# SkylerGao/MC_NeRF

Hardware: AMD Instinct MI355X
Metric: train rays/sec (coarse+fine, 64+128 samples) (higher is better)
Workload: dtype f16x3h; 1 GPU; Ball_Lego-shaped 110-view 800x800, coarse 4x128 @64 + fine 8x256 @128-grid, GLOBAL_OPTIM stage, fwd+bwd+allreduce+RAdam; precision=f16x3h, parallelism=dp1

## Files before the change

### mc_nerf_amd/csrc/mcnerf_16.h

```cpp
#pragma once
#include "mcnerf_common.h"

#define MCN16_SLAB 16
#define MCN16_RING (128 / MCN16_SLAB)
#define MCN16_AHEAD (MCN16_RING - 2)
#define MCN16_PPW (MCN16_SLAB / 8)
#define MCN16_WAVES 8
#define MCN16_ROWS (32 * MCN16_WAVES)
#define MCN16_ENCKS 4

struct Mcn16Part { int src, ld, col0, out_real, con_real, ksteps, map; };
static inline __host__ __device__ int mcn16_map_enc(int map) { return map >= 1 && map <= MCN_NFREQ; }
struct Mcn16Seg { int first_frag, tiles, transposed; Mcn16Part a, b; };
#define MCN16_MAXSEG 24
struct Mcn16Stream { int nseg, total_frags; Mcn16Seg seg[MCN16_MAXSEG]; };

static inline int mcn16_pad(int frags) { return (frags + MCN16_SLAB - 1) / MCN16_SLAB * MCN16_SLAB; }

static inline void mcn16_add(Mcn16Stream& st, int tiles, int transposed, Mcn16Part a, Mcn16Part b) {
    Mcn16Seg& s = st.seg[st.nseg++];
    s.first_frag = st.total_frags; s.tiles = tiles; s.transposed = transposed; s.a = a; s.b = b;
    st.total_frags += mcn16_pad(tiles * (a.ksteps + b.ksteps));
}

static inline Mcn16Stream mcn16_fwd_stream(const McnLayout& L) {
    Mcn16Stream st; st.nseg = 0; st.total_frags = 0;
    const int W = L.width, NT = W / 32, KS = W / 16;
    const int ME = L.nfreq == MCN_NFREQ ? 0 : L.nfreq, MS = L.sh_deg == 2 ? 0 : 16 + L.sh_deg;
    const Mcn16Part none = {0, 0, 0, 0, 0, 0, 0};
    mcn16_add(st, NT, 0, Mcn16Part{L.pW[0], L.nenc, 0, W, MCN_ENC, MCN16_ENCKS, ME}, none);
    for (int l = 1; l < L.depth; ++l) {
        if (l == L.skip) mcn16_add(st, NT, 0, Mcn16Part{L.pW[l], W + L.nenc, 0, W, MCN_ENC, MCN16_ENCKS, ME},
                                   Mcn16Part{L.pW[l], W + L.nenc, L.nenc, W, W, KS, 0});
        else mcn16_add(st, NT, 0, Mcn16Part{L.pW[l], W, 0, W, W, KS, 0}, none);
    }
    mcn16_add(st, NT, 0, Mcn16Part{L.pWs1, W, 0, W, W, KS, 0}, none);
    mcn16_add(st, NT, 0, Mcn16Part{L.pWc1, W, 0, W, W, KS, 0}, none);
    mcn16_add(st, 1, 0, Mcn16Part{L.pWc2, W, 0, MCN_NSH, W, KS, MS}, none);
    return st;
}
static inline Mcn16Stream mcn16_bwd_stream(const McnLayout& L) {
    Mcn16Stream st; st.nseg = 0; st.total_frags = 0;
    const int W = L.width, NT = W / 32, KS = W / 16;
    const int ME = L.nfreq == MCN_NFREQ ? 0 : L.nfreq, MS = L.sh_deg == 2 ? 0 : 16 + L.sh_deg;
    const Mcn16Part none = {0, 0, 0, 0, 0, 0, 0};
    mcn16_add(st, NT, 1, Mcn16Part{L.pWs1, W, 0, W, W, KS, 0}, none);
    mcn16_add(st, NT, 1, Mcn16Part{L.pWc2, W, 0, W, MCN_NSH, 2, MS}, none);
    mcn16_add(st, NT, 1, Mcn16Part{L.pWc1, W, 0, W, W, KS, 0}, none);
    for (int l = L.depth - 1; l >= 1; --l) {
        const int ld = (l == L.skip) ? W + L.nenc : W;
        if (l == L.skip) mcn16_add(st, 2, 1, Mcn16Part{L.pW[l], ld, 0, MCN_ENC, W, KS, ME}, none);
        mcn16_add(st, NT, 1, Mcn16Part{L.pW[l], ld, (l == L.skip) ? L.nenc : 0, W, W, KS, 0}, none);
    }
    mcn16_add(st, 2, 1, Mcn16Part{L.pW[0], L.nenc, 0, MCN_ENC, W, KS, ME}, none);
    return st;
}

static inline long long mcn16_cap_tiles(long long capacity) { return (capacity + MCN16_ROWS - 1) / MCN16_ROWS * MCN16_WAVES; }
static inline size_t mcn16_slot_bytes(long long capacity, int width) { return (size_t)mcn16_cap_tiles(capacity) * (width / 16) * 1024; }
static inline int mcn16_mask_words(int width) { return width >= 64 ? width / 64 : 1; }
static inline size_t mcn16_mask_slot_bytes(long long capacity, int width) { return (size_t)mcn16_cap_tiles(capacity) * 64 * 4 * mcn16_mask_words(width); }
static inline size_t mcn16_enc_bytes(long long capacity) { return (size_t)mcn16_cap_tiles(capacity) * MCN16_ENCKS * 1024; }
static inline size_t mcn16_dsh_bytes(long long capacity) { return (size_t)mcn16_cap_tiles(capacity) * 2 * 1024; }

static inline bool mcn16_is_bf16(int dtype) { return dtype == 1; }
static inline bool mcn16_x3_chain(int dtype) { return dtype == 2 || dtype == 3; }
static inline bool mcn16_hi_planes_only(int dtype) { return dtype == 3; }

struct Mcn16FwdArgs {
    McnLayout lay;
    const float* params;
    const void* packed;
    int stream_slabs;
    int dtype;
    const float* rays_o; const float* rays_d; const float* zgrid; const float* jitter; const float* barf_w;
    const int2* idx; const int* count; int max_rows; int n_rays, S;
    float* out;
    void* act_ws; size_t slot_bytes;
    void* enc_ws;
    unsigned* mask_ws; size_t mask_slot_words;
    void* sh_ws;
    int z_stride = 0;
};
hipError_t mcn16_launch_fwd(const Mcn16FwdArgs& a, hipStream_t st);

struct Mcn16BwdArgs {
    McnLayout lay;
    const float* params;
    const void* packed;
    int stream_slabs;
    int dtype;
    const float* rays_o; const float* rays_d; const float* zgrid; const float* jitter; const float* barf_w;
    const int2* idx; const int* count; int max_rows; int n_rays, S;
    const float* out; const float* d_out;
    const unsigned* mask_ws; size_t mask_slot_words;
    const void* enc_ws;
    const void* sh_ws;
    void* dy_ws; size_t slot_bytes;
    void* dsh_ws;
    float* d_rays_o; float* d_rays_d;
    const unsigned* gmax_bits;
    int z_stride = 0;
};
hipError_t mcn16_launch_bwd(const Mcn16BwdArgs& a, hipStream_t st);

struct Mcn16DwArgs {
    McnLayout lay;
    int dtype;
    const int* count; int rows;
    const void* act_ws; const void* enc_ws; const void* dy_ws; const void* dsh_ws;
    size_t slot_bytes;
    float* grads;
    const unsigned* gmax_bits;
    float x_scale;
};
hipError_t mcn16_launch_dw(const Mcn16DwArgs& a, hipStream_t st);

struct Dw16Seg {
    const char* dY; int ksn;
    const char* X;  int ksk;
    const char* X2; int ksk2;
    int n_lo, n_real;
    int col, k_real;
    int col2, k_real2;
    float* dW; int ldw;
    float* db;
    int kmap, kmap2, nmap;
};
#define MCN16_DW_MAXSEG 15

template <class Job>
static inline bool mcn16_dw_job(const Mcn16DwArgs& a, Job& job) {
    const McnLayout& L = a.lay;
    const int W = L.width, D = L.depth, KS = W / 16;
    const int ME = L.nfreq == MCN_NFREQ ? 0 : L.nfreq, MS = L.sh_deg == 2 ? 0 : 16 + L.sh_deg;
    auto act = [&](int slot) { return reinterpret_cast<const char*>(a.act_ws) + (size_t)slot * a.slot_bytes; };
    auto dy = [&](int slot) { return reinterpret_cast<const char*>(a.dy_ws) + (size_t)slot * a.slot_bytes; };
    const char* dsh = reinterpret_cast<const char*>(a.dsh_ws);
    float* const g = a.grads;
    job.n = 0;
    if (D + 5 > MCN16_DW_MAXSEG) return false;
    auto add = [&](int shape, const char* dY, int ksn, int n_lo, int n_real, float* dW, int ldw, float* db, int nmap = 0) -> Dw16Seg& {
        Dw16Seg& s = job.seg[job.n];
        job.shape[job.n++] = shape;
        s = Dw16Seg{};
        s.dY = dY; s.ksn = ksn; s.n_lo = n_lo; s.n_real = n_real; s.dW = dW; s.ldw = ldw; s.db = db; s.nmap = nmap;
        return s;
    };
    auto input = [](Dw16Seg& s, const char* x, int ks, int col, int k_real, int kmap) {
        if (!s.X) { s.X = x; s.ksk = ks; s.col = col; s.k_real = k_real; s.kmap = kmap; }
        else { s.X2 = x; s.ksk2 = ks; s.col2 = col; s.k_real2 = k_real; s.kmap2 = kmap; }
    };
    auto hidden = [&](Dw16Seg& s, int slot, int col) { input(s, act(slot), KS, col, W, 0); };
    auto encoded = [&](Dw16Seg& s) { input(s, reinterpret_cast<const char*>(a.enc_ws), MCN16_ENCKS, 0, MCN_ENC, ME); };
    const bool merged = (W == 256 || W == 128);
    for (int l = 0; l < D; ++l) {
        const int ldw = mcn_layer_in(L, l);
        float* dWl = g + L.pW[l];
        float* dbl = g + L.pB[l];
        if (l == 0) encoded(add(1, dy(l), KS, 0, W, dWl, ldw, dbl));
        else if (l == L.skip && merged) {
            Dw16Seg& s = add(3, dy(l), KS, 0, W, dWl, ldw, dbl);
            hidden(s, l - 1, L.nenc);
            encoded(s);
// ... 155 lines not shown
```

### mc_nerf_amd/csrc/mcnerf_x3.h

```cpp
#pragma once
#include "mcnerf_16.h"

#define MCNX3_SW 256.0f
#define MCNX3_SX 8.0f
#define MCNX3_SLABF 8
#define MCNX3_PF 2

#define MCNX3_WIDE_MIN 128
static inline constexpr int mcnx3_waves(int width) { return width >= MCNX3_WIDE_MIN ? 4 : 8; }

static inline int mcnx3_pad(int frags) { return (frags + MCNX3_SLABF - 1) / MCNX3_SLABF * MCNX3_SLABF; }
static inline Mcn16Stream mcnx3_repad(Mcn16Stream st) {
    int total = 0;
    for (int s = 0; s < st.nseg; ++s) {
        st.seg[s].first_frag = total;
        total += mcnx3_pad(st.seg[s].tiles * (st.seg[s].a.ksteps + st.seg[s].b.ksteps));
    }
    st.total_frags = total;
    return st;
}
static inline Mcn16Stream mcnx3_fwd_stream(const McnLayout& L) { return mcnx3_repad(mcn16_fwd_stream(L)); }
static inline Mcn16Stream mcnx3_bwd_stream(const McnLayout& L) { return mcnx3_repad(mcn16_bwd_stream(L)); }

static inline size_t mcnx3_slot_bytes(long long capacity, int width) { return 2 * mcn16_slot_bytes(capacity, width); }
static inline size_t mcnx3_enc_bytes(long long capacity) { return 2 * mcn16_enc_bytes(capacity); }
static inline size_t mcnx3_sh_bytes(long long capacity) { return (size_t)mcn16_cap_tiles(capacity) * 4096; }
static inline size_t mcnx3_dsh_bytes(long long capacity) { return 2 * mcn16_dsh_bytes(capacity); }

hipError_t mcnx3_launch_fwd(const Mcn16FwdArgs& a, hipStream_t st);
hipError_t mcnx3_launch_bwd(const Mcn16BwdArgs& a, hipStream_t st);
hipError_t mcnx3_launch_dw(const Mcn16DwArgs& a, hipStream_t st);
hipError_t mcnx3_launch_pack(const McnLayout& L, const float* params, void* packed_fwd, void* packed_bwd, unsigned* range_flags, hipStream_t st);

#ifdef __HIPCC__
typedef float f32x2_t __attribute__((ext_vector_type(2)));

__device__ __forceinline__ void mcnx3_split2(float a, float b, unsigned& hi, unsigned& lo) {
    const f16x2_t h = __builtin_convertvector((f32x2_t){a, b}, f16x2_t);
    const f32x2_t back = __builtin_convertvector(h, f32x2_t);
    const f16x2_t l = __builtin_convertvector((f32x2_t){a - back[0], b - back[1]}, f16x2_t);
    hi = __builtin_bit_cast(unsigned, h);
    lo = __builtin_bit_cast(unsigned, l);
}
__device__ __forceinline__ float mcnx3_val(unsigned hi, unsigned lo, int e) {
    const f16x2_t h = __builtin_bit_cast(f16x2_t, hi), l = __builtin_bit_cast(f16x2_t, lo);
    return (float)h[e] + (float)l[e];
}
template <int HI>
__device__ __forceinline__ float mcnx3_residual(float v, unsigned hw) {
    float r;
    if (HI) asm("v_fma_mix_f32 %0, %1, -1.0, %2 op_sel:[1,0,0] op_sel_hi:[1,0,0]" : "=v"(r) : "v"(hw), "v"(v));
    else asm("v_fma_mix_f32 %0, %1, -1.0, %2 op_sel_hi:[1,0,0]" : "=v"(r) : "v"(hw), "v"(v));
    return r;
}
__device__ __forceinline__ float mcnx3_relu(float x) {
    const int i = __builtin_bit_cast(int, x);
    return __builtin_bit_cast(float, i > 0 ? i : 0);
}
__device__ __forceinline__ f32x16 mcnx3_mfma(const u32x4_t& a, const u32x4_t& b, const f32x16& c) {
    return __builtin_amdgcn_mfma_f32_32x32x16_f16(__builtin_bit_cast(f16x8_t, a), __builtin_bit_cast(f16x8_t, b), c, 0, 0, 0);
}
__device__ __forceinline__ void mcnx3_mfma3(f32x16& acc, const u32x4_t& ah, const u32x4_t& al, const u32x4_t& bh, const u32x4_t& bl) {
    acc = mcnx3_mfma(al, bh, acc);
    acc = mcnx3_mfma(ah, bl, acc);
    acc = mcnx3_mfma(ah, bh, acc);
}

__device__ __forceinline__ void mcnx3_dma16(const char* ubase, unsigned voff, unsigned lds_dst) {
    unsigned keep;
    asm volatile("s_mov_b32 %0, m0\n\ts_mov_b32 m0, %3\n\ts_nop 0\n\tglobal_load_lds_dwordx4 %1, %2\n\ts_mov_b32 m0, %0"
                 : "=&s"(keep) : "v"(voff), "s"(ubase), "s"(lds_dst) : "memory");
}
template <int PPW>
__device__ __forceinline__ void mcnx3_ring_issue(Mcn16Ring& r) {
    const char* s = r.ubase + (size_t)r.src_slab * (MCN16_SLAB * 1024);
    const unsigned d = r.lds_base + r.issue_slot * (MCN16_SLAB * 1024) + r.lds_piece;
#pragma unroll
    for (int i = 0; i < PPW; ++i) mcnx3_dma16(s + i * 1024, r.voff, d + i * 1024);
    r.src_slab = (r.src_slab + 1 == r.n_slabs) ? 0 : r.src_slab + 1;
    r.issue_slot = (r.issue_slot + 1) & (MCN16_RING - 1);
}
template <int PPW>
__device__ __forceinline__ void mcnx3_ring_sync(Mcn16Ring& r) {
    asm volatile("s_waitcnt vmcnt(%0)\n\ts_barrier" ::"n"(PPW * (MCN16_AHEAD - 1)) : "memory");
    r.next_off = r.sync_slot * (MCN16_SLAB * 1024);
    r.sync_slot = (r.sync_slot + 1) & (MCN16_RING - 1);
    mcnx3_ring_issue<PPW>(r);
}
template <int PPW>
__device__ __forceinline__ void mcnx3_ring_start(Mcn16Ring& r, char* ring_lds, const void* packed, int n_slabs, int wave, int lane) {
    r.ubase = reinterpret_cast<const char*>(packed) + (PPW * wave) * 1024;
    r.voff = lane * 16;
    r.src = nullptr;
    r.lds_piece = (PPW * wave) * 1024;
    r.lds_base = (unsigned)reinterpret_cast<size_t>((mcn16_lds_ptr_t)ring_lds);
    r.src_slab = 0; r.n_slabs = n_slabs; r.issue_slot = 0; r.sync_slot = 0; r.next_off = 0;
#pragma unroll
    for (int i = 0; i < MCN16_AHEAD; ++i) mcnx3_ring_issue<PPW>(r);
    mcnx3_ring_sync<PPW>(r);
}
template <int F>
__host__ __device__ constexpr int mcnx3_sync_at(int q) {
    return (MCNX3_SLABF * q + MCNX3_SLABF - MCNX3_PF) < (F - 1) ? (MCNX3_SLABF * q + MCNX3_SLABF - MCNX3_PF) : (F - 1);
}
template <int F, int PPW>
__device__ __forceinline__ void mcnx3_before_mfma(Mcn16Ring& r, Mcn16Cursor& c, int f) {
    if ((f & (MCNX3_SLABF - 1)) == 0) c.cur = r.next_off;
    if (f == mcnx3_sync_at<F>(f / MCNX3_SLABF)) mcnx3_ring_sync<PPW>(r);
}
#define MCNX3_DMA_STEP 2
template <int PPW>
__device__ __forceinline__ void mcnx3_ring_piece(Mcn16Ring& r, int i) {
    switch (i) {
        case 0: asm volatile("global_load_lds_dwordx4 %0, %1" ::"v"(r.voff), "s"(r.piece_base) : "memory"); break;
        case 1: asm volatile("global_load_lds_dwordx4 %0, %1 offset:1024" ::"v"(r.voff), "s"(r.piece_base) : "memory"); break;
        case 2: asm volatile("global_load_lds_dwordx4 %0, %1 offset:2048" ::"v"(r.voff), "s"(r.piece_base) : "memory"); break;
        default: asm volatile("global_load_lds_dwordx4 %0, %1 offset:3072" ::"v"(r.voff), "s"(r.piece_base) : "memory"); break;
    }
}
template <int F, int PPW>
__device__ __forceinline__ void mcnx3_before_mfma_spread(Mcn16Ring& r, Mcn16Cursor& c, int f) {
    static_assert(PPW <= 4, "immediate offsets of the refill pieces");
    if ((f & (MCNX3_SLABF - 1)) == 0) c.cur = r.next_off;
    if (f == mcnx3_sync_at<F>(f / MCNX3_SLABF)) {
        asm volatile("s_waitcnt vmcnt(%0)\n\ts_barrier" ::"n"(PPW * (MCN16_AHEAD - 1)) : "memory");
        r.next_off = r.sync_slot * (MCN16_SLAB * 1024);
        r.sync_slot = (r.sync_slot + 1) & (MCN16_RING - 1);
        r.piece_base = r.ubase + (size_t)r.src_slab * (MCN16_SLAB * 1024);
        asm volatile("s_mov_b32 m0, %0" ::"s"(r.lds_base + r.issue_slot * (MCN16_SLAB * 1024) + r.lds_piece) : "memory");
        r.src_slab = (r.src_slab + 1 == r.n_slabs) ? 0 : r.src_slab + 1;
        r.issue_slot = (r.issue_slot + 1) & (MCN16_RING - 1);
    }
}
template <int F, int PPW>
__device__ __forceinline__ void mcnx3_gap_dma(Mcn16Ring& r, int gap) {
    constexpr int NQ = (F + MCNX3_SLABF - 1) / MCNX3_SLABF;
#pragma unroll
    for (int q = 0; q < NQ; ++q)
#pragma unroll
        for (int i = 0; i < PPW; ++i)
            if (gap == 3 * mcnx3_sync_at<F>(q) + 1 + MCNX3_DMA_STEP * i) mcnx3_ring_piece<PPW>(r, i);
}
template <int F, int PPW>
__device__ __forceinline__ void mcnx3_layer_end(Mcn16Ring& r) {
    constexpr int NQ = (F + MCNX3_SLABF - 1) / MCNX3_SLABF;
#pragma unroll
    for (int q = 0; q < NQ; ++q)
#pragma unroll
        for (int i = 0; i < PPW; ++i)
            if (3 * mcnx3_sync_at<F>(q) + 1 + MCNX3_DMA_STEP * i >= 3 * F) mcnx3_ring_piece<PPW>(r, i);
}
__device__ __forceinline__ unsigned mcnx3_frag_off(const Mcn16Ring& r, const Mcn16Cursor& c, int f_now, int f) {
    const bool next = (f / MCNX3_SLABF) != (f_now / MCNX3_SLABF);
    return (next ? r.next_off : c.cur) + (f & (MCNX3_SLABF - 1)) * 2048;
}

__device__ __forceinline__ void mcnx3_encode_values(const float (&p)[3], const float (&bw)[MCN_NFREQ], float (&E)[64]) {
    E[0] = p[0]; E[1] = p[1]; E[2] = p[2]; E[63] = 0.f;
#pragma unroll
    for (int a = 0; a < 3; ++a) {
        float S[MCN_NFREQ], C[MCN_NFREQ];
        mcn_sincos_octaves<MCN_NFREQ>(p[a], S, C);
#pragma unroll
        for (int f = 0; f < MCN_NFREQ; ++f) {
            E[3 + 20 * a + f] = S[f] * bw[f];
            E[3 + 20 * a + 10 + f] = C[f] * bw[f];
        }
    }
}
#endif
```

### mc_nerf_amd/csrc/mlp_x3_bwd.hip

```cpp
#include "mcnerf_x3.h"
#include "mcnerf_launch.h"

#define MCNX3_BWD_PREF_MINW 256
#include <cstdlib>

template <int W>
struct BwdX3Smem {
    static constexpr int WAVES = mcnx3_waves(W);
    static constexpr int oW2 = MCN16_RING * MCN16_SLAB * 1024;
    static constexpr int oBarf = oW2 + W * 4;
    static constexpr int MW = W >= 64 ? W / 64 : 1;
    static constexpr int oMask = oBarf + 16 * 4;
    static constexpr int oIdx = oMask + WAVES * 3 * MW * 256;
    static constexpr int oIn = oIdx + WAVES * 256;
    static constexpr int total = oIn + (W >= 256 ? WAVES * 16 * 256 : 0);
};

template <int W, int KSTEPS, int NTILES, int MODE, int PPW, bool HI>
__device__ __forceinline__ void mcnx3_bwd_seg(Mcn16Ring& ring, char* smem, int lane,
                                              const u32x4_t (&inh)[W / 16], const u32x4_t (&inl)[W / 16],
                                              u32x4_t (&outh)[W / 16], u32x4_t (&outl)[W / 16],
                                              const unsigned (&mk)[W >= 64 ? W / 64 : 1], f32x16 (&acc2)[2], char* save_lane) {
    constexpr int KS = W / 16, F = NTILES * KSTEPS, G = 3 * KSTEPS;
    constexpr bool EPI = MODE != 3;
    constexpr int NIT = EPI ? (MODE == 0 ? 16 : 20) : 0;
    constexpr int START = (G >= NIT + 8) ? 3 : 0;
    constexpr int IPG = EPI ? (NIT + (G - START) - 1) / (G - START) : 1;
    constexpr int LASTA = EPI ? START + 14 / IPG : 0;
    constexpr int SBASE = START + 16, SSTR = (G - SBASE) / 4 > 0 ? (G - SBASE) / 4 : 1;
    constexpr bool STAG = (MODE == 1 || MODE == 2) && IPG == 1 && (G - SBASE) / 4 >= 2;
    constexpr int NITG = STAG ? 16 : NIT;
    constexpr int INIT_G = (G - 8) > LASTA ? (G - 8) : LASTA;
    constexpr int INIT_N = (INIT_G + 3 <= G - 1) ? 4 : 1;
    Mcn16Cursor cur;
    u32x4_t afh[MCNX3_PF], afl[MCNX3_PF];
    f32x16 acc[2];
    float v0 = 0.f, v1 = 0.f;
    unsigned wkeep = 0u;
    auto acc_init = [&](f32x16& a, int t, int q) {
        if (MODE == 2) {
            const f16x8_t h8 = __builtin_bit_cast(f16x8_t, outh[2 * t + (q >> 1)]), l8 = __builtin_bit_cast(f16x8_t, outl[2 * t + (q >> 1)]);
#pragma unroll
            for (int e = 0; e < 4; ++e) a[4 * q + e] = ((float)h8[4 * (q & 1) + e] + (float)l8[4 * (q & 1) + e]) * MCNX3_SW;
        } else {
#pragma unroll
            for (int e = 0; e < 4; ++e) a[4 * q + e] = 0.f;
        }
    };
    auto item = [&](const f32x16& a, int t, int i) {
        if (i < 16) {
            const int p = i >> 1;
            const unsigned bits = MODE != 0 ? ((mk[t >> 1] >> (8 * (t & 1) + 7 - p)) & 0x00010001u) : 0u;
            if ((i & 1) == 0) {
                v0 = a[2 * p] * (1.0f / MCNX3_SW);
                v1 = a[2 * p + 1] * (1.0f / MCNX3_SW);
                const unsigned w = Mcn16T<false>::pack(v0, v1);
                wkeep = w;
                outh[2 * t + (p >> 2)][p & 3] = MODE != 0 ? mcn16_pkmul(w, bits) : w;
            } else {
                const unsigned w = Mcn16T<false>::pack(mcnx3_residual<0>(v0, wkeep), mcnx3_residual<1>(v1, wkeep));
                outl[2 * t + (p >> 2)][p & 3] = MODE != 0 ? mcn16_pkmul(w, bits) : w;
            }
        } else {
            const int k = i - 16, s = 2 * t + (k & 1);
            if (k < 2) mcn16_ws_store(outh[s], reinterpret_cast<u32x4_t*>(save_lane + s * 1024));
            else if (!HI) mcn16_ws_store(outl[s], reinterpret_cast<u32x4_t*>(save_lane + (KS + s) * 1024));
        }
    };
    cur.cur = ring.next_off;
#pragma unroll
    for (int i = 0; i < MCNX3_PF; ++i)
        if (i < F) {
            afh[i] = *reinterpret_cast<const u32x4_t*>(smem + ring.next_off + i * 2048 + lane * 16);
            afl[i] = *reinterpret_cast<const u32x4_t*>(smem + ring.next_off + i * 2048 + 1024 + lane * 16);
        }
    if (EPI) {
#pragma unroll
        for (int q = 0; q < 4; ++q) acc_init(acc[0], 0, q);
    }
#pragma unroll
    for (int t = 0; t < NTILES; ++t) {
#pragma unroll
        for (int s = 0; s < KSTEPS; ++s) {
            const int f = t * KSTEPS + s;
            mcnx3_before_mfma_spread<F, PPW>(ring, cur, f);
            const u32x4_t a_h = afh[f % MCNX3_PF], a_l = afl[f % MCNX3_PF];
            if (f + MCNX3_PF < F) {
                const unsigned o = mcnx3_frag_off(ring, cur, f, f + MCNX3_PF) + lane * 16;
                afh[f % MCNX3_PF] = *reinterpret_cast<const u32x4_t*>(smem + o);
                afl[f % MCNX3_PF] = *reinterpret_cast<const u32x4_t*>(smem + o + 1024);
            }
#pragma unroll
            for (int g = 0; g < 3; ++g) {
                const int gap = 3 * s + g;
                if (EPI && t > 0 && gap >= START) {
#pragma unroll
                    for (int i = (gap - START) * IPG; i < (gap - START + 1) * IPG; ++i)
                        if (i < NITG) item(acc[(t - 1) & 1], t - 1, i);
                    if (STAG && gap >= SBASE && (gap - SBASE) / SSTR < 4 && (gap - SBASE) % SSTR == 0)
                        item(acc[(t - 1) & 1], t - 1, 16 + (gap - SBASE) / SSTR);
                }
                if (EPI && t + 1 < NTILES && gap >= INIT_G && gap < INIT_G + INIT_N) {
#pragma unroll
                    for (int q = 0; q < 4; ++q)
                        if (INIT_N == 1 || q == gap - INIT_G) acc_init(acc[(t + 1) & 1], t + 1, q);
                }
                mcnx3_gap_dma<F, PPW>(ring, 3 * f + g);
                __builtin_amdgcn_sched_barrier(0);
                if (EPI) acc[t & 1] = mcnx3_mfma(g == 0 ? a_l : a_h, g == 1 ? inl[s] : inh[s], acc[t & 1]);
                else acc2[t & 1] = mcnx3_mfma(g == 0 ? a_l : a_h, g == 1 ? inl[s] : inh[s], acc2[t & 1]);
                __builtin_amdgcn_sched_barrier(0);
            }
        }
    }
    mcnx3_layer_end<F, PPW>(ring);
    if (EPI) {
#pragma unroll
        for (int i = 0; i < NIT; ++i) item(acc[(NTILES - 1) & 1], NTILES - 1, i);
    }
}

template <int W, bool HI>
__global__ __launch_bounds__(64 * mcnx3_waves(W), mcnx3_waves(W) / 4) void mlp_x3_bwd_kernel(Mcn16BwdArgs a) {
    using SM = BwdX3Smem<W>;
    constexpr int PL = HI ? 1 : 2;
    constexpr int WAVES = mcnx3_waves(W), ROWS = 32 * WAVES, PPW = 16 / WAVES;
    constexpr int NT = W / 32, KS = W / 16, MW = W >= 64 ? W / 64 : 1;
    extern __shared__ __attribute__((aligned(16))) char smem[];
    const int tid = threadIdx.x, lane = tid & 63, wave = __builtin_amdgcn_readfirstlane(tid >> 6);
    const int m = lane & 31, h = lane >> 5;
    const int D = a.lay.depth, skip = a.lay.skip;
    const long long total = a.count ? (long long)min(*a.count, a.max_rows) : (long long)a.n_rays * a.S;
    if ((long long)blockIdx.x * ROWS >= total) return;

    float* sw2 = reinterpret_cast<float*>(smem + SM::oW2);
    for (int i = tid; i < W; i += 64 * WAVES) sw2[i] = a.params[a.lay.pWs2 + i];
    float* sbarf = reinterpret_cast<float*>(smem + SM::oBarf);
    if (tid < MCN_NFREQ) sbarf[tid] = a.barf_w[tid];
    const float gmax = __uint_as_float(*a.gmax_bits);
    const float sg = mcn16_grad_scale(gmax);
    const float inv_sg = 1.0f / sg;
    __syncthreads();

    struct In { int ray; float zg, jit; f32x4 o, go; float dx, dy, dz, ox, oy, oz; };
    auto gather = [&](int ray, int j) -> In {
        In r;
        r.ray = ray;
        r.zg = a.zgrid[ray * a.z_stride + j];
        r.jit = a.jitter ? a.jitter[ray] : 0.f;
        const size_t addr = (size_t)ray * a.S + j;
        r.o = *reinterpret_cast<const f32x4*>(a.out + addr * 4);
        r.go = *reinterpret_cast<const f32x4*>(a.d_out + addr * 4);
        r.dx = a.rays_d[ray * 3]; r.dy = a.rays_d[ray * 3 + 1]; r.dz = a.rays_d[ray * 3 + 2];
        r.ox = a.rays_o[ray * 3]; r.oy = a.rays_o[ray * 3 + 1]; r.oz = a.rays_o[ray * 3 + 2];
        return r;
    };
    auto row_of = [&](long long pass_) -> long long {
        const long long g_ = (pass_ * WAVES + wave) * 32 + m;
        return g_ < total ? g_ : total - 1;
    };
    constexpr bool PREFB = W >= MCNX3_BWD_PREF_MINW;
    constexpr int SLABS_FULL = (W / 32) * (W / 16) / MCNX3_SLABF;
    constexpr int SLABS_ENC = (2 * (W / 16) + MCNX3_SLABF - 1) / MCNX3_SLABF;
    constexpr int N_IDX = PPW * (2 * SLABS_FULL - 1) < 63 ? PPW * (2 * SLABS_FULL - 1) : 63;
    constexpr int N_TOP = PPW * (SLABS_FULL + SLABS_ENC - 1) < 63 ? PPW * (SLABS_FULL + SLABS_ENC - 1) : 63;
    const unsigned in_lds = (unsigned)reinterpret_cast<size_t>((mcn16_lds_ptr_t)smem) + SM::oIn + wave * (16 * 256);
    const float* in_rd = reinterpret_cast<const float*>(smem + SM::oIn + wave * (16 * 256)) + lane;
    auto gather_dma = [&](int ray, int j) {
        mcn16_dma4(a.zgrid + ray * a.z_stride + j, in_lds);
        if (a.jitter) mcn16_dma4(a.jitter + ray, in_lds + 256);
        const size_t addr = ((size_t)ray * a.S + j) * 4;
#pragma unroll
        for (int c = 0; c < 4; ++c) {
            mcn16_dma4(a.out + addr + c, in_lds + (2 + c) * 256);
            mcn16_dma4(a.d_out + addr + c, in_lds + (6 + c) * 256);
        }
#pragma unroll
        for (int c = 0; c < 3; ++c) {
            mcn16_dma4(a.rays_d + ray * 3 + c, in_lds + (10 + c) * 256);
            mcn16_dma4(a.rays_o + ray * 3 + c, in_lds + (13 + c) * 256);
        }
    };
    auto read_in = [&](int ray) -> In {
        In r;
        r.ray = ray;
        r.zg = in_rd[0];
        r.jit = a.jitter ? in_rd[64] : 0.f;
        r.o = f32x4{in_rd[2 * 64], in_rd[3 * 64], in_rd[4 * 64], in_rd[5 * 64]};
        r.go = f32x4{in_rd[6 * 64], in_rd[7 * 64], in_rd[8 * 64], in_rd[9 * 64]};
        r.dx = in_rd[10 * 64]; r.dy = in_rd[11 * 64]; r.dz = in_rd[12 * 64];
        r.ox = in_rd[13 * 64]; r.oy = in_rd[14 * 64]; r.oz = in_rd[15 * 64];
        return r;
    };
    In cur;
    int ray_n = 0;
    {
        const long long gc0 = row_of(blockIdx.x);
        int ray0, j0;
        if (a.idx) { const int2 rj = a.idx[gc0]; ray0 = rj.x; j0 = rj.y; }
        else { ray0 = (int)(gc0 / a.S); j0 = (int)(gc0 - (long long)ray0 * a.S); }
        if (PREFB) { gather_dma(ray0, j0); ray_n = ray0; }
        else cur = gather(ray0, j0);
    }

    Mcn16Ring ring;
    mcnx3_ring_start<PPW>(ring, smem, a.packed, a.stream_slabs, wave, lane);
    const float* w2_h = sw2 + 4 * h;
    const unsigned idx_lds = (unsigned)reinterpret_cast<size_t>((mcn16_lds_ptr_t)smem) + SM::oIdx + wave * 256;

    constexpr bool MASK_DMA = W >= MCNX3_BWD_PREF_MINW;
    const unsigned mlds = ring.lds_base + SM::oMask + wave * (3 * MW * 256);
    auto mask_issue = [&](const unsigned* mask_lane, int slot, int buf) {
        if (MASK_DMA) {
#pragma unroll
            for (int i = 0; i < MW; ++i) mcn16_dma4(mask_lane + (size_t)slot * a.mask_slot_words + i, mlds + (buf * MW + i) * 256);
        }
    };
    auto mask_read = [&](const unsigned* mask_lane, unsigned (&mk)[MW], int buf, int slot) {
#pragma unroll
        for (int i = 0; i < MW; ++i) {
            if (MASK_DMA) mk[i] = *reinterpret_cast<const unsigned*>(smem + SM::oMask + wave * (3 * MW * 256) + (buf * MW + i) * 256 + lane * 4);
            else mk[i] = mask_lane[(size_t)slot * a.mask_slot_words + i];
        }
    };
    auto buf_of = [&](int slot) { return (D + 1 - slot) % 3; };
    auto mask_lane_of = [&](long long pass_) { return a.mask_ws + ((size_t)(pass_ * WAVES + wave) * 64 + lane) * MW; };
    unsigned mk0_s[MW], mk0_c[MW], mk0_t[MW];
    {
        const unsigned* ml0 = mask_lane_of(blockIdx.x);
        mask_issue(ml0, D, 0); mask_issue(ml0, D + 1, 1); mask_issue(ml0, D - 1, 2);
        if (!MASK_DMA) { mask_read(ml0, mk0_s, 0, D); mask_read(ml0, mk0_c, 1, D + 1); mask_read(ml0, mk0_t, 2, D - 1); }
        asm volatile("s_waitcnt vmcnt(0)" ::: "memory");
    }

    for (long long pass = blockIdx.x; pass * ROWS < total; pass += gridDim.x) {
        const long long tile = pass * WAVES + wave;
        const long long g = tile * 32 + m;
        const bool valid = g < total;
        const unsigned* mask_lane = mask_lane_of(pass);
        char* dy_lane = reinterpret_cast<char*>(a.dy_ws) + (size_t)tile * (PL * KS) * 1024 + lane * 16;
        if (PREFB) {
            asm volatile("s_waitcnt vmcnt(%0)" ::"n"(N_TOP) : "memory");
            cur = read_in(ray_n);
        }
        const int ray = cur.ray;
        unsigned mk_s[MW], mk_c[MW], mk_t[MW];
        float zv = cur.zg;
        if (a.jitter) zv = __fadd_rn(zv, cur.jit);
        const f32x4 o = cur.o;
        f32x4 go = cur.go;
        if (!valid) go = f32x4{0.f, 0.f, 0.f, 0.f};
        const float x = cur.dx, y = cur.dy, z = cur.dz;
        float p[3];
        p[0] = __fadd_rn(cur.ox, __fmul_rn(x, zv));
        p[1] = __fadd_rn(cur.oy, __fmul_rn(y, zv));
        p[2] = __fadd_rn(cur.oz, __fmul_rn(z, zv));
        float bas[9];
        mcn_sh_basis(x, y, z, bas);
        float dpre[3];
#pragma unroll
        for (int c = 0; c < 3; ++c) dpre[c] = go[1 + c] * o[1 + c] * (1.f - o[1 + c]) * sg;
        const float dsg = go[0] * sg;
        u32x4_t dshh[2], dshl[2];
#pragma unroll
        for (int s = 0; s < 2; ++s)
#pragma unroll
            for (int d = 0; d < 4; ++d) {
                float v[2];
#pragma unroll
                for (int u = 0; u < 2; ++u) {
                    const int n0 = mcn16_chan(s, 0, 2 * d + u), n1 = n0 + 4;
                    const float va = n0 < MCN_NSH ? dpre[n0 / 9] * bas[n0 % 9] : (n0 == MCN_NSH ? dsg : 0.f);
                    const float vb = n1 < MCN_NSH ? dpre[n1 / 9] * bas[n1 % 9] : (n1 == MCN_NSH ? dsg : 0.f);
                    v[u] = h ? vb : va;
                }
                unsigned wh, wl;
                mcnx3_split2(v[0], v[1], wh, wl);
                dshh[s][d] = wh; dshl[s][d] = wl;
            }
        {
            char* e = reinterpret_cast<char*>(a.dsh_ws) + (size_t)tile * (PL * 2) * 1024 + lane * 16;
            mcn16_ws_store(dshh[0], reinterpret_cast<u32x4_t*>(e));
            mcn16_ws_store(dshh[1], reinterpret_cast<u32x4_t*>(e + 1024));
            if (!HI) {
                mcn16_ws_store(dshl[0], reinterpret_cast<u32x4_t*>(e + 2048));
                mcn16_ws_store(dshl[1], reinterpret_cast<u32x4_t*>(e + 3072));
            }
        }

        if (MASK_DMA) mask_read(mask_lane, mk_s, 0, D);
        else {
#pragma unroll
            for (int i = 0; i < MW; ++i) { mk_s[i] = mk0_s[i]; mk_c[i] = mk0_c[i]; mk_t[i] = mk0_t[i]; }
        }
        const long long pass_n = pass + gridDim.x;
        if (a.idx) {
            const long long gn = (pass_n * WAVES + wave) * 32 + (lane >> 1);
            mcn16_dma4(reinterpret_cast<const int*>(a.idx) + 2 * (gn < total ? gn : total - 1) + (lane & 1), idx_lds);
        }
        const bool want_rays = a.d_rays_o || a.d_rays_d;
        f32x4 shs[4];
#pragma unroll
        for (int q = 0; q < 4; ++q) shs[q] = f32x4{0.f, 0.f, 0.f, 0.f};
        if (PREFB && want_rays) {
#pragma unroll
            for (int q = 0; q < 4; ++q)
                shs[q] = *reinterpret_cast<const f32x4*>(reinterpret_cast<const char*>(a.sh_ws) + (size_t)tile * 4096 + q * 1024 + lane * 16);
        }
        u32x4_t xah[KS], xal[KS], xbh[KS], xbl[KS];
        f32x16 denc[2];
#pragma unroll
        for (int t = 0; t < 2; ++t)
#pragma unroll
            for (int e = 0; e < 16; ++e) denc[t][e] = 0.f;
#pragma unroll
        for (int s = 0; s < KS; ++s) {
            const f32x4 wa = *reinterpret_cast<const f32x4*>(w2_h + 16 * s), wb = *reinterpret_cast<const f32x4*>(w2_h + 16 * s + 8);
            const int t = s >> 1;
#pragma unroll
            for (int d = 0; d < 4; ++d) {
                const float va = (d < 2 ? wa[2 * d] : wb[2 * d - 4]) * dsg, vb = (d < 2 ? wa[2 * d + 1] : wb[2 * d - 3]) * dsg;
                const int i = 4 * (s & 1) + d;
                const unsigned bits = (mk_s[t >> 1] >> (8 * (t & 1) + 7 - i)) & 0x00010001u;
                unsigned wh, wl;
                mcnx3_split2(va, vb, wh, wl);
                xah[s][d] = mcn16_pkmul(wh, bits);
                xal[s][d] = mcn16_pkmul(wl, bits);
            }
            mcn16_ws_store(xah[s], reinterpret_cast<u32x4_t*>(dy_lane + (size_t)D * a.slot_bytes + s * 1024));
            if (!HI) mcn16_ws_store(xal[s], reinterpret_cast<u32x4_t*>(dy_lane + (size_t)D * a.slot_bytes + (KS + s) * 1024));
        }
        if (D >= 2) mask_issue(mask_lane, D - 2, buf_of(D - 2));
        unsigned mpend[MW];
        if (!MASK_DMA && D >= 2) mask_read(mask_lane, mpend, 0, D - 2);
        mcnx3_bwd_seg<W, KS, NT, 0, PPW, HI>(ring, smem, lane, xah, xal, xbh, xbl, mk_s, denc, nullptr);
        if (MASK_DMA) mask_read(mask_lane, mk_c, 1, D + 1);
        {
            u32x4_t dih[KS], dil[KS];
            dih[0] = dshh[0]; dih[1] = dshh[1]; dil[0] = dshl[0]; dil[1] = dshl[1];
            mcnx3_bwd_seg<W, 2, NT, 1, PPW, HI>(ring, smem, lane, dih, dil, xah, xal, mk_c, denc, dy_lane + (size_t)(D + 1) * a.slot_bytes);
        }
        if (D >= 3) mask_issue(mask_lane, D - 3, buf_of(D - 3));
        if (MASK_DMA) mask_read(mask_lane, mk_t, 2, D - 1);
        mcnx3_bwd_seg<W, KS, NT, 2, PPW, HI>(ring, smem, lane, xah, xal, xbh, xbl, mk_t, denc, dy_lane + (size_t)(D - 1) * a.slot_bytes);
        auto trunk_masks = [&](int l) {
            if (MASK_DMA) {
                if (l >= 3) mask_issue(mask_lane, l - 3, buf_of(l - 3));
                mask_read(mask_lane, mk_t, buf_of(l - 1), l - 1);
            } else {
#pragma unroll
                for (int i = 0; i < MW; ++i) mk_t[i] = mpend[i];
                if (l >= 2) mask_read(mask_lane, mpend, 0, l - 2);
            }
            if (l == 1 && pass_n * ROWS < total) {
                const unsigned* mln = mask_lane_of(pass_n);
                mask_issue(mln, D, 0); mask_issue(mln, D + 1, 1); mask_issue(mln, D - 1, 2);
                if (!MASK_DMA) { mask_read(mln, mk0_s, 0, D); mask_read(mln, mk0_c, 1, D + 1); mask_read(mln, mk0_t, 2, D - 1); }
            }
        };
        auto next_rows = [&]() {
            asm volatile("s_waitcnt vmcnt(%0)" ::"n"(N_IDX) : "memory");
            int rn, jn;
            if (a.idx) {
                const int2 rj = *reinterpret_cast<const int2*>(smem + SM::oIdx + wave * 256 + m * 8);
                rn = rj.x; jn = rj.y;
            } else {
                const long long gn = row_of(pass_n);
                rn = (int)(gn / a.S); jn = (int)(gn - (long long)rn * a.S);
            }
            gather_dma(rn, jn);
            ray_n = rn;
        };
        for (int l = D - 1; l >= 1; l -= 2) {
            if (PREFB && l == 1) next_rows();
            trunk_masks(l);
            if (l == skip) mcnx3_bwd_seg<W, KS, 2, 3, PPW, HI>(ring, smem, lane, xbh, xbl, xah, xal, mk_t, denc, nullptr);
            mcnx3_bwd_seg<W, KS, NT, 1, PPW, HI>(ring, smem, lane, xbh, xbl, xah, xal, mk_t, denc, dy_lane + (size_t)(l - 1) * a.slot_bytes);
            if (l - 1 >= 1) {
                if (PREFB && l - 1 == 1) next_rows();
                trunk_masks(l - 1);
                if (l - 1 == skip) mcnx3_bwd_seg<W, KS, 2, 3, PPW, HI>(ring, smem, lane, xah, xal, xbh, xbl, mk_t, denc, nullptr);
                mcnx3_bwd_seg<W, KS, NT, 1, PPW, HI>(ring, smem, lane, xah, xal, xbh, xbl, mk_t, denc, dy_lane + (size_t)(l - 2) * a.slot_bytes);
            } else {
#pragma unroll
                for (int s = 0; s < KS; ++s) { xbh[s] = xah[s]; xbl[s] = xal[s]; }
            }
        }
        In nxt = cur;
        if (PREFB && D < 2) {
            next_rows();
        }
        if (!PREFB) {
            int rn, jn;
            if (a.idx) {
                const int2 rj = *reinterpret_cast<const int2*>(smem + SM::oIdx + wave * 256 + m * 8);
                rn = rj.x; jn = rj.y;
            } else {
                const long long gn = row_of(pass_n);
                rn = (int)(gn / a.S); jn = (int)(gn - (long long)rn * a.S);
            }
            nxt = gather(rn, jn);
        }
        if (!PREFB && want_rays) {
#pragma unroll
            for (int q = 0; q < 4; ++q)
                shs[q] = *reinterpret_cast<const f32x4*>(reinterpret_cast<const char*>(a.sh_ws) + (size_t)tile * 4096 + q * 1024 + lane * 16);
        }
        mcnx3_bwd_seg<W, KS, 2, 3, PPW, HI>(ring, smem, lane, xbh, xbl, xah, xal, mk_t, denc, nullptr);
        auto settle = [&]() {
            if (PREFB && D >= 2) return;
            asm volatile("s_waitcnt vmcnt(0)" ::: "memory");
            asm volatile("" : "+v"(nxt.ray), "+v"(nxt.zg), "+v"(nxt.jit), "+v"(nxt.o), "+v"(nxt.go));
            asm volatile("" : "+v"(nxt.dx), "+v"(nxt.dy), "+v"(nxt.dz), "+v"(nxt.ox), "+v"(nxt.oy), "+v"(nxt.oz));
            if (!MASK_DMA) {
#pragma unroll
                for (int i = 0; i < MW; ++i) asm volatile("" : "+v"(mk0_s[i]), "+v"(mk0_c[i]), "+v"(mk0_t[i]));
            }
        };

        if (want_rays) {
            auto dch = [&](int ch) -> float {
                const int hh = (ch >> 2) & 1;
                const float v = denc[ch >> 5][4 * ((ch >> 3) & 3) + (ch & 3)];
                return (h == hh) ? v : 0.f;
            };
            float dpos[3];
#pragma unroll
            for (int ax = 0; ax < 3; ++ax) {
                float acc = dch(ax);
                float S[MCN_NFREQ], C[MCN_NFREQ];
                mcn_sincos_octaves<MCN_NFREQ>(p[ax], S, C);
#pragma unroll
                for (int f = 0; f < MCN_NFREQ; ++f) {
                    const float k = (float)(1 << f) * sbarf[f];
                    acc = fmaf(k * C[f], dch(3 + 20 * ax + f), acc);
                    acc = fmaf(-k * S[f], dch(3 + 20 * ax + 10 + f), acc);
                }
                dpos[ax] = acc * (1.0f / MCNX3_SW);
            }
            float ddir[3] = {0.f, 0.f, 0.f};
            {
                const float C1 = 0.4886025119029199f, C20 = 1.0925484305920792f, C22 = 0.31539156525252005f, C24 = 0.5462742152960396f;
                const float gx[9] = {0.f, 0.f, 0.f, -C1, C20 * y, 0.f, -2.f * C22 * x, -C20 * z, 2.f * C24 * x};
                const float gy[9] = {0.f, -C1, 0.f, 0.f, C20 * x, -C20 * z, -2.f * C22 * y, 0.f, -2.f * C24 * y};
                const float gz[9] = {0.f, 0.f, C1, 0.f, 0.f, -C20 * y, 4.f * C22 * z, -C20 * x, 0.f};
#pragma unroll
                for (int r = 0; r < 16; ++r) {
                    const float v = shs[r >> 2][r & 3];
                    const int n0 = 8 * (r >> 2) + (r & 3), n1 = n0 + 4;
                    const float kx = h ? (n1 < MCN_NSH ? dpre[n1 / 9] * gx[n1 % 9] : 0.f) : (n0 < MCN_NSH ? dpre[n0 / 9] * gx[n0 % 9] : 0.f);
                    const float ky = h ? (n1 < MCN_NSH ? dpre[n1 / 9] * gy[n1 % 9] : 0.f) : (n0 < MCN_NSH ? dpre[n0 / 9] * gy[n0 % 9] : 0.f);
                    const float kz = h ? (n1 < MCN_NSH ? dpre[n1 / 9] * gz[n1 % 9] : 0.f) : (n0 < MCN_NSH ? dpre[n0 / 9] * gz[n0 % 9] : 0.f);
                    ddir[0] = fmaf(kx, v, ddir[0]); ddir[1] = fmaf(ky, v, ddir[1]); ddir[2] = fmaf(kz, v, ddir[2]);
                }
            }
            float red[6];
#pragma unroll
            for (int c = 0; c < 3; ++c) {
                const float dp = dpos[c] + __shfl_xor(dpos[c], 32);
                const float dd = ddir[c] + __shfl_xor(ddir[c], 32);
                red[c] = dp * inv_sg;
                red[3 + c] = (dp * zv + dd) * inv_sg;
            }
            settle();
            const int rkey = valid ? ray : -1;
            const int rprev = __shfl_up(rkey, 1, 32);
            int head = (m == 0 || rprev != rkey) ? 1 : 0;
#pragma unroll
            for (int off = 1; off < 32; off <<= 1) {
                const int hup = __shfl_up(head, off, 32);
                const bool take = (m >= off) && !head;
#pragma unroll
                for (int c = 0; c < 6; ++c) {
                    const float up = __shfl_up(red[c], off, 32);
                    red[c] += take ? up : 0.f;
                }
                if (m >= off) head |= hup;
            }
            const int rnext = __shfl_down(rkey, 1, 32);
            if (h == 0 && valid && (m == 31 || rnext != rkey)) {
#pragma unroll
                for (int c = 0; c < 3; ++c) {
                    if (a.d_rays_o) atomicAdd(a.d_rays_o + ray * 3 + c, red[c]);
                    if (a.d_rays_d) atomicAdd(a.d_rays_d + ray * 3 + c, red[3 + c]);
                }
            }
        }
        if (!want_rays) settle();
// ... 13 lines not shown
```

### mc_nerf_amd/csrc/pack16.hip

```cpp
#include "mcnerf_16.h"

__device__ __forceinline__ void mcn16_range_watch(const float (&v)[8], float limit, unsigned* flags, int seg) {
    float m = 0.f;
#pragma unroll
    for (int j = 0; j < 8; ++j) m = fmaxf(m, fabsf(v[j])) + (v[j] != v[j] ? __builtin_inff() : 0.f);
    if (!(m <= limit)) atomicOr(flags + seg, 1u);
}

__device__ __forceinline__ float mcn16_pack_src(const float* __restrict__ params, const Mcn16Part& p, int transposed, int o, int c) {
    if (p.map) {
        if (mcn16_map_enc(p.map)) { if (transposed) o = mcn_enc_col(o, p.map); else c = mcn_enc_col(c, p.map); }
        else { if (transposed) c = mcn_sh_row(c, p.map - 16); else o = mcn_sh_row(o, p.map - 16); }
        if (o < 0 || c < 0) return 0.f;
    }
    return transposed ? params[p.src + (size_t)c * p.ld + p.col0 + o] : params[p.src + (size_t)o * p.ld + p.col0 + c];
}

template <bool BF>
__global__ void pack16_kernel(Mcn16Stream sf, Mcn16Stream sb, const float* __restrict__ params, char* __restrict__ pf, char* __restrict__ pb, unsigned* flags) {
    const int gid = blockIdx.x * blockDim.x + threadIdx.x;
    const int nf = sf.total_frags * 64, nb = sb.total_frags * 64;
    if (gid >= nf + nb) return;
    const bool bwd = gid >= nf;
    const Mcn16Stream& st = bwd ? sb : sf;
    const int id = bwd ? gid - nf : gid;
    const int frag = id >> 6, lane = id & 63;
    const int i = lane & 31, h = lane >> 5;
    int s = 0;
    while (s + 1 < st.nseg && frag >= st.seg[s + 1].first_frag) ++s;
    const Mcn16Seg sg = st.seg[s];
    const int loc = frag - sg.first_frag;
    const int per_tile = sg.a.ksteps + sg.b.ksteps;
    const int t = loc / per_tile, ks = loc - t * per_tile;
    float v[8];
#pragma unroll
    for (int j = 0; j < 8; ++j) v[j] = 0.f;
    if (t < sg.tiles) {
        const bool inb = ks >= sg.a.ksteps;
        const Mcn16Part p = inb ? sg.b : sg.a;
        const int kk = inb ? ks - sg.a.ksteps : ks;
        const int o = 32 * t + i;
#pragma unroll
        for (int j = 0; j < 8; ++j) {
            const int c = mcn16_chan(kk, h, j);
            if (o < p.out_real && c < p.con_real) v[j] = mcn16_pack_src(params, p, sg.transposed, o, c);
        }
    }
    if (flags && !bwd) mcn16_range_watch(v, BF ? 3.0e38f : 65504.f, flags, s);
    u32x4_t w;
#pragma unroll
    for (int d = 0; d < 4; ++d) w[d] = Mcn16T<BF>::pack(v[2 * d], v[2 * d + 1]);
    *reinterpret_cast<u32x4_t*>((bwd ? pb : pf) + (size_t)id * 16) = w;
}

hipError_t mcn16_launch_pack(const McnLayout& L, const float* params, void* packed_fwd, void* packed_bwd, int bf16, unsigned* flags, hipStream_t st) {
    const Mcn16Stream sf = mcn16_fwd_stream(L), sb = mcn16_bwd_stream(L);
    const int total = (sf.total_frags + sb.total_frags) * 64;
    const int threads = 256, grid = (total + threads - 1) / threads;
    if (bf16) hipLaunchKernelGGL(pack16_kernel<true>, dim3(grid), dim3(threads), 0, st, sf, sb, params, (char*)packed_fwd, (char*)packed_bwd, flags);
    else hipLaunchKernelGGL(pack16_kernel<false>, dim3(grid), dim3(threads), 0, st, sf, sb, params, (char*)packed_fwd, (char*)packed_bwd, flags);
    return hipGetLastError();
}

#include "mcnerf_x3.h"
__global__ void packx3_kernel(Mcn16Stream sf, Mcn16Stream sb, const float* __restrict__ params, char* __restrict__ pf, char* __restrict__ pb, unsigned* flags) {
    const int gid = blockIdx.x * blockDim.x + threadIdx.x;
    const int nf = sf.total_frags * 64, nb = sb.total_frags * 64;
    if (gid >= nf + nb) return;
    const bool bwd = gid >= nf;
    const Mcn16Stream& st = bwd ? sb : sf;
    const int id = bwd ? gid - nf : gid;
    const int frag = id >> 6, lane = id & 63;
    const int i = lane & 31, h = lane >> 5;
    int s = 0;
    while (s + 1 < st.nseg && frag >= st.seg[s + 1].first_frag) ++s;
    const Mcn16Seg sg = st.seg[s];
    const int loc = frag - sg.first_frag;
    const int per_tile = sg.a.ksteps + sg.b.ksteps;
    const int t = loc / per_tile, ks = loc - t * per_tile;
    float v[8];
#pragma unroll
    for (int j = 0; j < 8; ++j) v[j] = 0.f;
    if (t < sg.tiles) {
        const bool inb = ks >= sg.a.ksteps;
        const Mcn16Part p = inb ? sg.b : sg.a;
        const int kk = inb ? ks - sg.a.ksteps : ks;
        const int o = 32 * t + i;
#pragma unroll
        for (int j = 0; j < 8; ++j) {
            const int c = mcn16_chan(kk, h, j);
            if (o < p.out_real && c < p.con_real) v[j] = mcn16_pack_src(params, p, sg.transposed, o, c);
        }
    }
    if (flags && !bwd) mcn16_range_watch(v, 65504.f / MCNX3_SW, flags, s);
    u32x4_t wh, wl;
#pragma unroll
    for (int d = 0; d < 4; ++d) {
        unsigned a, b;
        mcnx3_split2(v[2 * d] * MCNX3_SW, v[2 * d + 1] * MCNX3_SW, a, b);
        wh[d] = a; wl[d] = b;
    }
    char* dst = (bwd ? pb : pf) + (size_t)frag * 2048 + lane * 16;
    *reinterpret_cast<u32x4_t*>(dst) = wh;
    *reinterpret_cast<u32x4_t*>(dst + 1024) = wl;
}

hipError_t mcnx3_launch_pack(const McnLayout& L, const float* params, void* packed_fwd, void* packed_bwd, unsigned* flags, hipStream_t st) {
    const Mcn16Stream sf = mcnx3_fwd_stream(L), sb = mcnx3_bwd_stream(L);
    const int total = (sf.total_frags + sb.total_frags) * 64;
    const int threads = 256, grid = (total + threads - 1) / threads;
    hipLaunchKernelGGL(packx3_kernel, dim3(grid), dim3(threads), 0, st, sf, sb, params, (char*)packed_fwd, (char*)packed_bwd, flags);
    return hipGetLastError();
}
```

Before: 1.083 million rays/s.

## Fold sigma-head weights into packed bwd matrix, use one-plane mask B operand

In the backward sigma.0^T segment, the per-row sigma weight (w2 scaled) is folded into the packed weight matrix at pack time via a new per-part scale index. The B operand then becomes just the 0/1 ReLU mask (exact in one fp16 plane), so the split-precision product drops from three MFMAs to two per k-step and the epilogue rescales by dsg. This removes one MFMA per step and the hi/lo split of the B operand, at the cost of extra pack work and reliance on dsg being a scalar per row block.

```diff
diff --git a/mc_nerf_amd/csrc/mcnerf_16.h b/mc_nerf_amd/csrc/mcnerf_16.h
--- a/mc_nerf_amd/csrc/mcnerf_16.h
+++ b/mc_nerf_amd/csrc/mcnerf_16.h
@@ -9,7 +9,7 @@
 #define MCN16_ROWS (32 * MCN16_WAVES)
 #define MCN16_ENCKS 4
 
-struct Mcn16Part { int src, ld, col0, out_real, con_real, ksteps, map; };
+struct Mcn16Part { int src, ld, col0, out_real, con_real, ksteps, map; int scale = -1; };
 static inline __host__ __device__ int mcn16_map_enc(int map) { return map >= 1 && map <= MCN_NFREQ; }
 struct Mcn16Seg { int first_frag, tiles, transposed; Mcn16Part a, b; };
 #define MCN16_MAXSEG 24
diff --git a/mc_nerf_amd/csrc/mcnerf_x3.h b/mc_nerf_amd/csrc/mcnerf_x3.h
--- a/mc_nerf_amd/csrc/mcnerf_x3.h
+++ b/mc_nerf_amd/csrc/mcnerf_x3.h
@@ -20,7 +20,11 @@
     return st;
 }
 static inline Mcn16Stream mcnx3_fwd_stream(const McnLayout& L) { return mcnx3_repad(mcn16_fwd_stream(L)); }
-static inline Mcn16Stream mcnx3_bwd_stream(const McnLayout& L) { return mcnx3_repad(mcn16_bwd_stream(L)); }
+static inline Mcn16Stream mcnx3_bwd_stream(const McnLayout& L) {
+    Mcn16Stream st = mcn16_bwd_stream(L);
+    st.seg[0].a.scale = L.pWs2;
+    return mcnx3_repad(st);
+}
 
 static inline size_t mcnx3_slot_bytes(long long capacity, int width) { return 2 * mcn16_slot_bytes(capacity, width); }
 static inline size_t mcnx3_enc_bytes(long long capacity) { return 2 * mcn16_enc_bytes(capacity); }
diff --git a/mc_nerf_amd/csrc/mlp_x3_bwd.hip b/mc_nerf_amd/csrc/mlp_x3_bwd.hip
--- a/mc_nerf_amd/csrc/mlp_x3_bwd.hip
+++ b/mc_nerf_amd/csrc/mlp_x3_bwd.hip
@@ -16,12 +16,15 @@
     static constexpr int total = oIn + (W >= 256 ? WAVES * 16 * 256 : 0);
 };
 
-template <int W, int KSTEPS, int NTILES, int MODE, int PPW, bool HI>
+template <int W, int KSTEPS, int NTILES, int MODE, int PPW, bool HI, bool BITB = false>
 __device__ __forceinline__ void mcnx3_bwd_seg(Mcn16Ring& ring, char* smem, int lane,
                                               const u32x4_t (&inh)[W / 16], const u32x4_t (&inl)[W / 16],
                                               u32x4_t (&outh)[W / 16], u32x4_t (&outl)[W / 16],
-                                              const unsigned (&mk)[W >= 64 ? W / 64 : 1], f32x16 (&acc2)[2], char* save_lane) {
-    constexpr int KS = W / 16, F = NTILES * KSTEPS, G = 3 * KSTEPS;
+                                              const unsigned (&mk)[W >= 64 ? W / 64 : 1], f32x16 (&acc2)[2], char* save_lane,
+                                              const float esc = 1.0f / MCNX3_SW) {
+    static_assert(!BITB || MODE == 0, "the one-plane B operand is the sigma.0^T segment's");
+    constexpr int MPS = BITB ? 2 : 3;
+    constexpr int KS = W / 16, F = NTILES * KSTEPS, G = MPS * KSTEPS;
     constexpr bool EPI = MODE != 3;
     constexpr int NIT = EPI ? (MODE == 0 ? 16 : 20) : 0;
     constexpr int START = (G >= NIT + 8) ? 3 : 0;
@@ -52,8 +55,8 @@
             const int p = i >> 1;
             const unsigned bits = MODE != 0 ? ((mk[t >> 1] >> (8 * (t & 1) + 7 - p)) & 0x00010001u) : 0u;
             if ((i & 1) == 0) {
-                v0 = a[2 * p] * (1.0f / MCNX3_SW);
-                v1 = a[2 * p + 1] * (1.0f / MCNX3_SW);
+                v0 = a[2 * p] * esc;
+                v1 = a[2 * p + 1] * esc;
                 const unsigned w = Mcn16T<false>::pack(v0, v1);
                 wkeep = w;
                 outh[2 * t + (p >> 2)][p & 3] = MODE != 0 ? mcn16_pkmul(w, bits) : w;
@@ -91,8 +94,8 @@
                 afl[f % MCNX3_PF] = *reinterpret_cast<const u32x4_t*>(smem + o + 1024);
             }
 #pragma unroll
-            for (int g = 0; g < 3; ++g) {
-                const int gap = 3 * s + g;
+            for (int g = 0; g < MPS; ++g) {
+                const int gap = MPS * s + g;
                 if (EPI && t > 0 && gap >= START) {
 #pragma unroll
                     for (int i = (gap - START) * IPG; i < (gap - START + 1) * IPG; ++i)
@@ -106,8 +109,9 @@
                         if (INIT_N == 1 || q == gap - INIT_G) acc_init(acc[(t + 1) & 1], t + 1, q);
                 }
                 mcnx3_gap_dma<F, PPW>(ring, 3 * f + g);
+                if (BITB && g == 1) mcnx3_gap_dma<F, PPW>(ring, 3 * f + 2);
                 __builtin_amdgcn_sched_barrier(0);
-                if (EPI) acc[t & 1] = mcnx3_mfma(g == 0 ? a_l : a_h, g == 1 ? inl[s] : inh[s], acc[t & 1]);
+                if (EPI) acc[t & 1] = mcnx3_mfma(g == 0 ? a_l : a_h, (!BITB && g == 1) ? inl[s] : inh[s], acc[t & 1]);
                 else acc2[t & 1] = mcnx3_mfma(g == 0 ? a_l : a_h, g == 1 ? inl[s] : inh[s], acc2[t & 1]);
                 __builtin_amdgcn_sched_barrier(0);
             }
@@ -315,25 +319,27 @@
             for (int e = 0; e < 16; ++e) denc[t][e] = 0.f;
 #pragma unroll
         for (int s = 0; s < KS; ++s) {
+            const int t = s >> 1;
+            u32x4_t dyh, dyl = {0u, 0u, 0u, 0u};
             const f32x4 wa = *reinterpret_cast<const f32x4*>(w2_h + 16 * s), wb = *reinterpret_cast<const f32x4*>(w2_h + 16 * s + 8);
-            const int t = s >> 1;
 #pragma unroll
             for (int d = 0; d < 4; ++d) {
-                const float va = (d < 2 ? wa[2 * d] : wb[2 * d - 4]) * dsg, vb = (d < 2 ? wa[2 * d + 1] : wb[2 * d - 3]) * dsg;
                 const int i = 4 * (s & 1) + d;
                 const unsigned bits = (mk_s[t >> 1] >> (8 * (t & 1) + 7 - i)) & 0x00010001u;
+                xah[s][d] = bits * 0x3C00u;
+                const float va = (d < 2 ? wa[2 * d] : wb[2 * d - 4]) * dsg, vb = (d < 2 ? wa[2 * d + 1] : wb[2 * d - 3]) * dsg;
                 unsigned wh, wl;
                 mcnx3_split2(va, vb, wh, wl);
-                xah[s][d] = mcn16_pkmul(wh, bits);
-                xal[s][d] = mcn16_pkmul(wl, bits);
-            }
-            mcn16_ws_store(xah[s], reinterpret_cast<u32x4_t*>(dy_lane + (size_t)D * a.slot_bytes + s * 1024));
-            if (!HI) mcn16_ws_store(xal[s], reinterpret_cast<u32x4_t*>(dy_lane + (size_t)D * a.slot_bytes + (KS + s) * 1024));
+                dyh[d] = mcn16_pkmul(wh, bits);
+                if (!HI) dyl[d] = mcn16_pkmul(wl, bits);
+            }
+            mcn16_ws_store(dyh, reinterpret_cast<u32x4_t*>(dy_lane + (size_t)D * a.slot_bytes + s * 1024));
+            if (!HI) mcn16_ws_store(dyl, reinterpret_cast<u32x4_t*>(dy_lane + (size_t)D * a.slot_bytes + (KS + s) * 1024));
         }
         if (D >= 2) mask_issue(mask_lane, D - 2, buf_of(D - 2));
         unsigned mpend[MW];
         if (!MASK_DMA && D >= 2) mask_read(mask_lane, mpend, 0, D - 2);
-        mcnx3_bwd_seg<W, KS, NT, 0, PPW, HI>(ring, smem, lane, xah, xal, xbh, xbl, mk_s, denc, nullptr);
+        mcnx3_bwd_seg<W, KS, NT, 0, PPW, HI, true>(ring, smem, lane, xah, xah, xbh, xbl, mk_s, denc, nullptr, dsg * (1.0f / MCNX3_SW));
         if (MASK_DMA) mask_read(mask_lane, mk_c, 1, D + 1);
         {
             u32x4_t dih[KS], dil[KS];
diff --git a/mc_nerf_amd/csrc/pack16.hip b/mc_nerf_amd/csrc/pack16.hip
--- a/mc_nerf_amd/csrc/pack16.hip
+++ b/mc_nerf_amd/csrc/pack16.hip
@@ -89,7 +89,10 @@
 #pragma unroll
         for (int j = 0; j < 8; ++j) {
             const int c = mcn16_chan(kk, h, j);
-            if (o < p.out_real && c < p.con_real) v[j] = mcn16_pack_src(params, p, sg.transposed, o, c);
+            if (o < p.out_real && c < p.con_real) {
+                v[j] = mcn16_pack_src(params, p, sg.transposed, o, c);
+                if (p.scale >= 0) v[j] = __fmul_rn(v[j], params[p.scale + c]);
+            }
         }
     }
     if (flags && !bwd) mcn16_range_watch(v, 65504.f / MCNX3_SW, flags, s);
```

New measurement: 1.093 million rays/s, median of 6. About the same (+0.9%).
